# qingqing-zijin/LEAD-YOLO

Hardware: AMD Instinct MI355X
Metric: images/sec (640x640) fwd+bwd (higher is better)
Workload: dtype bf16; 1 GPU; lead-yolo-s bs=64/gpu 3x640x640 bf16 full train step: uint8 batch -> train-mode forward (batch-statistics BN), ComputeLoss, HIP backward, clip 10, SGD-nesterov 3 groups, ModelEMA update (BASELINE.json configs[2]); random-init weights; global_batch=64, parallelism=dp1 (single GPU, no collective), world_size=1

## Files before the change

### include/lead_yolo_hip.h

```cpp
#ifndef LEAD_YOLO_HIP_H
#define LEAD_YOLO_HIP_H
#ifdef __cplusplus
extern "C" {
#endif

enum { LY_F32 = 0, LY_BF16 = 1 };
int ly_abi_version(void);
const char* ly_last_error(void);

int ly_mlpblock_fwd(const void* x , void* y , int n_img, int H, int W, int C, const void* wp, const void* w1,
                    const void* w2, const float* bn_scale, const float* bn_shift, double* stats, int dtype, void* stream);
int ly_mlpblock_fwd_describe(int n_img, int H, int W, int C, int dtype, int with_stats , char* name, int cap);
int ly_mlpblock_pconv(const void* x , void* z , int n_img, int H, int W, int C, const void* wp, int dtype, void* stream);
int ly_mlpblock_pconv_describe(int n_img, int H, int W, int C, int dtype, char* name, int cap);
int ly_mlpblock_bwd_ok(int C, int dtype);
long ly_mlpblock_bwd_slab_floats(int C);
int ly_mlpblock_bwd(const void* x , const void* dy , void* g , int n_img, int H, int W, int C, const void* wp, const void* w1,
                    const void* w2t, const void* w1t, const float* a, const float* b, const float* alpha, const float* kappa, const float* lambda,
                    double* stats, float* slab, long slab_floats, float* dw1, float* dw2, int pass, int dtype, void* stream);
int ly_mlpblock_bwd_describe(int n_img, int H, int W, int C, int dtype, int pass, char* name, int cap);
int ly_mlpblock_bwd_dx_ok(int C, int W, int dtype);
int ly_mlpblock_bwd_dx(const void* g , const void* dy , const void* x , void* dx , int n_img, int H, int W, int C, const void* wpt,
                       float* slab, long slab_floats, float* dwp, int lddw, int dw_ts, int dw_cs, int dtype, void* stream);
int ly_mlpblock_bwd_dx_describe(int n_img, int H, int W, int C, int dtype, int with_dw , char* name, int cap);
// ... 52 lines not shown
} LyConv3Params;

int ly_conv3x3_fwd(const LyConv3Params* p, void* stream);
int ly_conv3x3_describe(const LyConv3Params* p, char* name, int cap);


int ly_pool_hw(const void* x , int ldx, int n_img, int H, int W, int C, float* pool, int dtype, void* stream);
int ly_coordatt_mlp(const float* pool, int n_img, int H, int W, int C, int mip, const float* w1, const float* b1,
                    const float* sc, const float* sh, const float* wh, const float* bh, const float* ww, const float* bw, float* a_h,
                    float* a_w, void* stream);
int ly_coordatt_mlp_bwd(const float* pool, int n_img, int H, int W, int C, int mip, const float* w1, const float* b1,
                        const float* mean, const float* invstd, const float* gamma, const float* beta, const float* wh,
                        const float* ww, const float* a_h, const float* a_w, const float* da_h, const float* da_w, float* ws,
                        double* sums , float* dpool, float* dw1, float* dgamma, float* dbeta, float* dwh, float* dbh, float* dww,
                        float* dbw, int grads_f64 , void* stream);

int ly_coordatt_gate(const void* x , int ldx, int n_img, int H, int W, int C, const float* a_h, const float* a_w,
                     const void* res , int ldres, void* out , int ldo, int dtype, void* stream);

int ly_se_fwd(const void* x , int ldx, int n_img, int HW, int C, const float* wa, const float* wb, int R, float* part,
              int slices, float* ca, int dtype, void* stream);
int ly_rfcbam_stats(const void* x , int ldx, int n_img, int H, int W, int C, int k, int s, const float* wg,
                    const float* a1, const float* b1, int TH, int TW, float* mm, float* part, int slices, int dtype, void* stream);
int ly_rfcbam_stats_describe(const void* x , int ldx, int n_img, int H, int W, int C, int k, int s, const float* wg, const float* a1, const float* b1,
                             int TH, int TW, float* mm, float* part, int slices, int dtype, char* name, int cap);
int ly_colsum(const void* x , int ldx, int n_img, int HW, int C, float* part, int slices, int dtype, void* stream);
int ly_rfcbam_mid(const float* part, int slices, int C, int HW, const float* wa, const float* wb, int R, float* ca, int n_img,
                  const float* mm, int HK, int WK, const float* w18, float* rfa, void* stream);
int ly_rfa_map(const float* mm, int n_img, int HK, int WK, const float* w, float* rfa, void* stream);

// ... 196 lines not shown
int ly_tune_wgrad3(int on);
int ly_tune_wgrad1(int on);

int ly_up2_bwd(const void* d , int ldd, int n_img, int Hs, int Ws, int C, void* out , int ldo, int dtype, void* stream);
int ly_unpatch(const void* g , int n_img, int Ho, int Wo, int C, int ks, void* dx , int dtype, void* stream);
int ly_sum_rows(const float* src, long R, long C, long ld, float* dst, int accumulate, void* stream);
int ly_patch4_rows_u8(const unsigned char* img, int n_img, int C, int H, int W, void* rows , int dtype, void* stream);
int ly_patch4_wgrad_u8(const unsigned char* img, int n_img, int C, int H, int W, const void* du , int lddu, int N, float scale, float* slab,
                       long slab_floats, float* dw , int dtype, void* stream);
int ly_patch4_wgrad_u8_describe(const unsigned char* img, int n_img, int C, int H, int W, const void* du , int lddu, int N, float scale, float* slab,
                                long slab_floats, float* dw, int dtype, char* name, int cap);

int ly_coordatt_gate_bwd(const void* dout , int ldd, const void* x , int ldx, int n_img, int H, int W, int C, const float* a_h,
                         const float* a_w, void* dx , int lddx, float* da_h, float* da_w, int bands, int slabs, int dtype, void* stream);
int ly_pool_hw_bwd(const float* gp, int n_img, int H, int W, int C, void* dx , int lddx, int accumulate, int dtype, void* stream);
int ly_maxpool_arg(const void* x , int ldx, int n_img, int H, int W, int C, int k, unsigned char* arg, int lda, int dtype, void* stream);
int ly_maxpool_gather(const unsigned char* arg, int lda, const float* d_up, int ldu, const void* d_own, int ldd, int own_dtype, int n_img, int H,
                      int W, int C, int k, void* out, int ldo, int out_dtype, void* stream);
int ly_sppf_bwd(const void* buf , int ldb, const void* d , int ldd, int n_img, int H, int W, int c, int k, void* out , int ldo, int dtype,
                void* stream);
int ly_mlp_dx(const void* dy , const void* g , const void* t , int ldt, long rows, int C, int c4, void* dx , int dtype, void* stream);
int ly_maxpool_bwd(const void* x , int ldx, const float* dy, int lddy, int n_img, int H, int W, int C, int k, float* dx, int lddx,
                   int dtype, void* stream);

int ly_rf_generate(const void* x , int ldx, int n_img, int H, int W, int C, int k, int s, const float* wg, void* ug , int dtype, void* stream);
int ly_rf_bwd_attn(int n_img, int H, int W, int C, int k, int s, const void* ug , const void* dcd , const float* ag, const float* bg,
                   const float* ca, const float* rfa, void* cd , float* d_rfa, float* gmax, float* d_ca, int dtype, void* stream);
int ly_rfa_bwd(const float* d_rfa, const float* rfa, const float* mm, const float* w18, int n_img, int Hk, int Wk, float* d_mm,
               float* dw18, int dw18_f64 , void* stream);
int ly_rf_bwd_relu(int n_img, int H, int W, int C, int k, int s, const void* ug , void* dcd , const float* ag, const float* bg,
// ... 110 lines not shown
```

### lead-yolo_amd/csrc/ly_attention.hip

```cpp
#include <float.h>

#include "ly_tile.hpp"
#include "ly_params.h"


template <typename T>
__global__ __launch_bounds__(LY_THREADS) void ly_pool_hw_kernel(const T* __restrict__ x, int ldx, int H, int W, int C,
                                                                 float* __restrict__ pool) {
  __shared__ f32x4 red[LY_THREADS];
  const int L = H + W;
  const int bid = ly_xcd_remap((int)blockIdx.x, (int)gridDim.x);
  const int n = bid / L, pos = bid - n * L;
  const int nc4 = C >> 2;
  const int tid = threadIdx.x;
  const int groups = LY_THREADS / nc4;
  const bool row = pos < H;
  const int len = row ? W : H;
  const long base = row ? ((long)n * H + pos) * W : ((long)n * H) * W + (pos - H);
  const long step = row ? 1 : W;
  const int c4 = tid % nc4, j0 = tid / nc4;
  f32x4 s = ly_zero4();
  if (j0 < groups) {
#pragma unroll 4
    for (int j = j0; j < len; j += groups) s += ly_ld4<T>(x + (base + j * step) * ldx + 4 * c4);
// ... 1231 lines not shown
                                                                                   n_img, H, W, C, Ho, Wo, s, mom)),
                                  "ly_rfcbam_tap_moments_kernel<%s>", ly_tname<T>()));
}

extern "C" int ly_rfcbam_tap_moments(const void* x, int ldx, int n_img, int H, int W, int C, int s, double* mom, int dtype, void* stream) {
  return tap_moments_entry(x, ldx, n_img, H, W, C, s, mom, dtype, LY_ON_STREAM(stream));
}

extern "C" int ly_rfcbam_tap_moments_describe(const void* x, int ldx, int n_img, int H, int W, int C, int s, double* mom, int dtype, char* name, int cap) {
  LY_CHECK(name && cap > 0, "rfcbam_tap_moments_describe: bad arguments");
  return tap_moments_entry(x, ldx, n_img, H, W, C, s, mom, dtype, LyOut{nullptr, name, cap});
}

__device__ __forceinline__ float ly_hswish_grad(float x) { return x <= -3.f ? 0.f : (x >= 3.f ? 1.f : (2.f * x + 3.f) * (1.f / 6.f)); }
#define LY_CA_STRIPES 32

template <int MIP, int NS>
__global__ __launch_bounds__(LY_THREADS) void ly_coordatt_mlp_bwd1_kernel(
    const float* __restrict__ pool, int n_img, int H, int W, int C, const float* __restrict__ w1, const float* __restrict__ b1,
    const float* __restrict__ mean, const float* __restrict__ invstd, const float* __restrict__ gamma, const float* __restrict__ beta,
    const float* __restrict__ wh, const float* __restrict__ ww, const float* __restrict__ a_h, const float* __restrict__ a_w,
    const float* __restrict__ da_h, const float* __restrict__ da_w, float* __restrict__ ws, double* __restrict__ sums, float* __restrict__ dzb) {
  const int tid = threadIdx.x, lane = tid & 63, wave = tid >> 6;
  const int L = H + W;
  const long R = (long)n_img * L;
  float s1 = 0.f, s2 = 0.f;
  static_assert(MIP == 8 || MIP == 16, "ly_coordatt_mlp_bwd1: MIP = 8 or 16");
  constexpr int LSTEP = 64 / MIP;
  const int mine = lane / LSTEP;
  const bool owner = (lane % LSTEP) == 0;
  const float b1m = b1[mine], meanm = mean[mine], invm = invstd[mine], gm = gamma[mine], bem = beta[mine];
  const long nw = (long)gridDim.x * 4;
  for (long r = (long)blockIdx.x * 4 + wave; r < R; r += nw) {
    const long n = r / L;
    const int pos = (int)(r - n * L);
    const bool isrow = pos < H;
    const long q = isrow ? n * H + pos : n * W + (pos - H);
    const float* wx = isrow ? wh : ww;
    const float* am = (isrow ? a_h : a_w) + q * C;
    const float* dam = (isrow ? da_h : da_w) + q * C;
    float y[MIP], d[MIP];
#pragma unroll
    for (int m = 0; m < MIP; ++m) { y[m] = 0.f; d[m] = 0.f; }
#pragma unroll
    for (int sl = 0; sl < NS; ++sl) {
      const int c = lane + 64 * sl;
      if (c < C) {
        const float pv = pool[r * C + c];
        const float av = am[c];
        const float dz = dam[c] * av * (1.f - av);
        dzb[r * C + c] = dz;
#pragma unroll
        for (int m = 0; m < MIP; ++m) {
          y[m] += w1[m * C + c] * pv;
          d[m] += dz * wx[c * MIP + m];
        }
      }
    }
    ly_reduce_scatter<MIP>(y, lane);
    ly_reduce_scatter<MIP>(d, lane);
    if (owner) {
      const float xh = (y[0] + b1m - meanm) * invm;
      const float y1 = gm * xh + bem;
      const float g = d[0] * ly_hswish_grad(y1);
      s1 += g;
// ... 91 lines not shown
    const int cl = e / NA, k = e - cl * NA;
    const int cc = blockIdx.x * 64 + cl;
    if (cc >= C) continue;
    const float v = red[e] + red[64 * NA + e] + red[2 * 64 * NA + e] + red[3 * 64 * NA + e];
    if (k < MIP) ly_gacc(dw1, k * C + cc, v, f64);
    else if (k < 2 * MIP) ly_gacc(dwh, cc * MIP + (k - MIP), v, f64);
    else if (k < 3 * MIP) ly_gacc(dww, cc * MIP + (k - 2 * MIP), v, f64);
    else if (k == 3 * MIP) ly_gacc(dbh, cc, v, f64);
    else ly_gacc(dbw, cc, v, f64);
  }
}

template <int MIP, int NS>
static void launch_coordatt_bwd(hipStream_t st, const float* pool, int n_img, int H, int W, int C, const float* w1, const float* b1, const float* mean,
                                const float* invstd, const float* gamma, const float* beta, const float* wh, const float* ww, const float* a_h,
                                const float* a_w, const float* da_h, const float* da_w, float* ws, double* sums, float* dpool, float* dw1,
                                float* dgamma, float* dbeta, float* dwh, float* dbh, float* dww, float* dbw, int f64) {
  const long R = (long)n_img * (H + W);
  long b1n = (R + 3) / 4;
  if (b1n > 1024) b1n = 1024;
  hipLaunchKernelGGL((ly_coordatt_mlp_bwd1_kernel<MIP, NS>), dim3((unsigned)b1n), dim3(LY_THREADS), 0, st, pool, n_img, H, W, C, w1, b1, mean, invstd, gamma,
                     beta, wh, ww, a_h, a_w, da_h, da_w, ws, sums, dpool);
  const int groups = (C + 63) / 64;
  long chunks = (96 + groups - 1) / groups;
  if (chunks > (R + 31) / 32) chunks = (R + 31) / 32;
  if (chunks < 1) chunks = 1;
  const long rpb = (R + chunks - 1) / chunks;
  chunks = (R + rpb - 1) / rpb;
  hipLaunchKernelGGL((ly_coordatt_mlp_bwd2_kernel<MIP>), dim3((unsigned)groups, (unsigned)chunks), dim3(LY_THREADS), 0, st, pool, n_img, H, W, C, rpb, w1,
                     gamma, invstd, ws, sums, dpool, dw1, dgamma, dbeta, dwh, dbh, dww, dbw, f64);
}

extern "C" int ly_coordatt_mlp_bwd(const float* pool, int n_img, int H, int W, int C, int mip, const float* w1, const float* b1,
                                   const float* mean, const float* invstd, const float* gamma, const float* beta, const float* wh,
                                   const float* ww, const float* a_h, const float* a_w, const float* da_h, const float* da_w, float* ws,
                                   double* sums, float* dpool, float* dw1, float* dgamma, float* dbeta, float* dwh, float* dbh,
                                   float* dww, float* dbw, int grads_f64, void* stream) {
  LY_CHECK(pool && w1 && b1 && mean && invstd && gamma && beta && wh && ww && a_h && a_w && da_h && da_w && ws && sums && dpool && dw1 &&
               dgamma && dbeta && dwh && dbh && dww && dbw, "coordatt_mlp_bwd: null pointer");
  LY_CHECK((mip == 8 || mip == 16) && C > 0 && C <= 512 && n_img > 0 && H > 0 && W > 0, "coordatt_mlp_bwd: built for mip 8 / 16 and C <= 512 (mip=%d C=%d)", mip, C);
  hipStream_t st = reinterpret_cast<hipStream_t>(stream);
#define LY_CA_BWD(MIP, NS) launch_coordatt_bwd<MIP, NS>(st, pool, n_img, H, W, C, w1, b1, mean, invstd, gamma, beta, wh, ww, a_h, a_w, da_h, da_w, ws, sums, \
                                                        dpool, dw1, dgamma, dbeta, dwh, dbh, dww, dbw, grads_f64)
  const int ns = (C + 63) / 64;
  if (mip == 8) {
    if (ns <= 1) LY_CA_BWD(8, 1); else if (ns <= 2) LY_CA_BWD(8, 2); else if (ns <= 4) LY_CA_BWD(8, 4); else LY_CA_BWD(8, 8);
  } else {
    if (ns <= 4) LY_CA_BWD(16, 4); else LY_CA_BWD(16, 8);
  }
#undef LY_CA_BWD
  LY_LAUNCH_CHECK();
  return 0;
}

__device__ __forceinline__ long ly_gw_index(int ch, int t, int e, int chunk, bool contiguous) {
  const int per = chunk >> 2;
  const int q = ch / chunk, r = ch - q * chunk;
  const int w = contiguous ? r / per : r & 3;
  const int j = contiguous ? r - w * per : r >> 2;
  const int p = j >> 1, ab = j & 1;
  return (((((long)q * 4 + w) * 9 + t) * (per >> 1) + p) * 10 + e) * 2 + ab;
}

__global__ __launch_bounds__(LY_THREADS) void ly_rfcbam_gen_prepare_kernel(
    const double* __restrict__ mom, int C, int KK, const float* __restrict__ gen_w, const float* __restrict__ gamma,
    const float* __restrict__ beta, float eps, float momentum, double count, float* __restrict__ running_mean,
    float* __restrict__ running_var, long* __restrict__ nbt, float* __restrict__ out8 , float* __restrict__ a1,
// ... 185 lines not shown
```

### lead-yolo_amd/csrc/ly_backward.hip

```cpp
#include "ly_tile.hpp"
#include "ly_params.h"

template <int ACT>
__device__ __forceinline__ f32x4 ly_dact4(const f32x4 v, const f32x4 dy) {
  f32x4 r;
#pragma unroll
  for (int i = 0; i < 4; ++i) {
    if (ACT == LY_ACT_RELU) {
      r[i] = v[i] > 0.f ? dy[i] : 0.f;
    } else if (ACT == LY_ACT_SILU) {
      const float s = ly_sigmoid(v[i]);
      r[i] = dy[i] * s * (1.f + v[i] * (1.f - s));
    } else {
      r[i] = dy[i];
    }
  }
  return r;
}

#ifndef LY_XCD_STREAM
#define LY_XCD_STREAM 1
#endif
#if LY_XCD_STREAM
#define LY_XCD_RANGE(total)                                                                                             \
// ... 451 lines not shown

extern "C" int ly_patch4_rows_u8(const unsigned char* img, int n_img, int C, int H, int W, void* rows, int dtype, void* stream) {
  LY_CHECK_DTYPE(dtype, "patch4_rows_u8");
  LY_CHECK(img && rows && n_img > 0 && C > 0 && C <= 16 && H > 0 && W > 0 && (H & 3) == 0 && (W & 3) == 0, "patch4_rows_u8: bad arguments");
  LY_CHECK(((uintptr_t)img & 3) == 0 && ((uintptr_t)rows & 15) == 0, "patch4_rows_u8: unaligned pointer");
  LY_CHECK((long)n_img * (H >> 2) < 65536, "patch4_rows_u8: too many patch rows");
  const dim3 grid((unsigned)(((W >> 2) + LY_P4_WO - 1) / LY_P4_WO), (unsigned)(n_img * (H >> 2)));
  LY_WITH_T(dtype, hipLaunchKernelGGL(ly_patch4_rows_u8_kernel<T>, grid, dim3(LY_THREADS), (size_t)LY_P4_WO * (16 * C + 8) * sizeof(T),
                                      reinterpret_cast<hipStream_t>(stream), img, C, H, W, reinterpret_cast<T*>(rows)));
  LY_LAUNCH_CHECK();
  return 0;
}

#define LY_CAG_RB 8
#define LY_CAG_MAXW 8
template <typename T>
__global__ __launch_bounds__(LY_THREADS) void ly_coordatt_gate_bwd_kernel(const T* __restrict__ dout, int ldd, const T* __restrict__ x,
                                                                           int ldx, int H, int W, int C, const float* __restrict__ a_h,
                                                                           const float* __restrict__ a_w, T* __restrict__ dx, int lddx,
                                                                           float* __restrict__ da_h, float* __restrict__ da_w, int bands, int slabs, long n_img) {
  __shared__ f32x4 red[LY_THREADS];
  const int nc4 = C >> 2, tid = threadIdx.x;
  const int groups = LY_THREADS / nc4;
  const int c4 = tid % nc4, g0 = tid / nc4;
  const int slab = blockIdx.x % slabs;
  const int bb = blockIdx.x / slabs;
  const long n = bb / bands;
  const int band = bb - (int)n * bands;
  const int w0 = slab * groups * LY_CAG_MAXW;
  const int h_lo = band * LY_CAG_RB, h_hi = h_lo + LY_CAG_RB < H ? h_lo + LY_CAG_RB : H;
  f32x4 accw[LY_CAG_MAXW], aw[LY_CAG_MAXW];
  bool okw[LY_CAG_MAXW];
  int wcl[LY_CAG_MAXW];
  const bool gok = g0 < groups;
#pragma unroll
// ... 11 lines not shown
    {
      const int c4c = gok ? c4 : 0;
      const f32x4 ah = ly_ldg4(a_h + nh * C + 4 * c4c);
      R4 dr[LY_CAG_MAXW], xr[LY_CAG_MAXW];
#pragma unroll
      for (int i = 0; i < LY_CAG_MAXW; ++i) {
        const long row = nh * W + wcl[i];
        dr[i] = ly_ldr4<T>(dout + row * ldd + 4 * c4c);
        xr[i] = ly_ldr4<T>(x + row * ldx + 4 * c4c);
      }
#pragma unroll
      for (int i = 0; i < LY_CAG_MAXW; ++i) {
        if (okw[i]) {
          const long row = nh * W + wcl[i];
          const f32x4 d = ly_r4_f32(dr[i]), xv = ly_r4_f32(xr[i]);
          ly_st4<T>(dx + row * lddx + 4 * c4, d * ah * aw[i]);
          const f32x4 t = d * xv;
          sh += t * aw[i];
          accw[i] += t * ah;
        }
      }
    }
    __syncthreads();
    red[tid] = sh;
    __syncthreads();
    if (g0 == 0) {
      for (int g = 1; g < groups; ++g) sh += red[g * nc4 + c4];
      ly_stg4(da_h + ((long)slab * n_img * H + nh) * C + 4 * c4, sh);
    }
  }
  if (g0 < groups) {
#pragma unroll
    for (int i = 0; i < LY_CAG_MAXW; ++i) {
      const int w = w0 + g0 + i * groups;
      if (w < W) {
        ly_stg4(da_w + ((long)band * n_img * W + n * W + w) * C + 4 * c4, accw[i]);
      }
    }
  }
}

extern "C" int ly_coordatt_gate_bwd(const void* dout, int ldd, const void* x, int ldx, int n_img, int H, int W, int C, const float* a_h,
                                    const float* a_w, void* dx, int lddx, float* da_h, float* da_w, int bands_in, int slabs_in, int dtype, void* stream) {
  LY_CHECK_DTYPE(dtype, "coordatt_gate_bwd");
  LY_CHECK(dout && x && a_h && a_w && dx && da_h && da_w, "coordatt_gate_bwd: null pointer");
  LY_CHECK((C & 3) == 0 && C <= 1024 && (ldd & 3) == 0 && (ldx & 3) == 0 && (lddx & 3) == 0, "coordatt_gate_bwd: C / ld must be multiples of 4");
  const int groups = LY_THREADS / (C >> 2);
  const int slabs = (W + groups * LY_CAG_MAXW - 1) / (groups * LY_CAG_MAXW);
  const int bands = (H + LY_CAG_RB - 1) / LY_CAG_RB;
  LY_CHECK(bands_in == bands && slabs_in == slabs, "coordatt_gate_bwd: the partial buffers are da_h [%d slabs][n][H][C] and da_w [%d bands][n][W][C] (got %d, %d)",
           slabs, bands, slabs_in, bands_in);
  LY_WITH_T(dtype, hipLaunchKernelGGL(ly_coordatt_gate_bwd_kernel<T>, dim3((unsigned)(n_img * bands * slabs)), dim3(LY_THREADS), 0, reinterpret_cast<hipStream_t>(stream),
                                      reinterpret_cast<const T*>(dout), ldd, reinterpret_cast<const T*>(x), ldx, H, W, C, a_h, a_w, reinterpret_cast<T*>(dx), lddx, da_h, da_w,
                                      bands, slabs, (long)n_img));
  LY_LAUNCH_CHECK();
  return 0;
}

template <typename T, bool ACC>
__global__ __launch_bounds__(LY_THREADS) void ly_pool_hw_bwd_kernel(const float* __restrict__ gp, int n_img, int H, int W, int C,
                                                                    T* __restrict__ dx, int lddx) {
  constexpr int VW = LyT<T>::VW, NQ = VW / 4;
  using RV = typename LyT<T>::RV;
  if ((C % VW) == 0 && (lddx % VW) == 0 && C / VW <= LY_THREADS) {
    const int ncv = C / VW, groups = LY_THREADS / ncv;
    const int cv = threadIdx.x % ncv, wl = threadIdx.x / ncv;
    if (wl >= groups) return;
    const int c = VW * cv;
    const float iw = 1.f / (float)W, ih = 1.f / (float)H;
// ... 40 lines not shown
}

extern "C" int ly_pool_hw_bwd(const float* gp, int n_img, int H, int W, int C, void* dx, int lddx, int accumulate, int dtype, void* stream) {
  LY_CHECK_DTYPE(dtype, "pool_hw_bwd");
  LY_CHECK(gp && dx && n_img > 0 && H > 0 && W > 0 && (C & 3) == 0 && (lddx & 3) == 0, "pool_hw_bwd: bad arguments");
  long nb = ly_ew_blocks((long)n_img * H * W * (C >> 2));
  if (nb > (long)n_img * H) nb = (long)n_img * H;
  const dim3 grid((unsigned)nb);
  if (accumulate) {
    LY_WITH_T(dtype, hipLaunchKernelGGL((ly_pool_hw_bwd_kernel<T, true>), grid, dim3(LY_THREADS), 0, reinterpret_cast<hipStream_t>(stream), gp, n_img, H, W, C,
                                        reinterpret_cast<T*>(dx), lddx));
  } else {
    LY_WITH_T(dtype, hipLaunchKernelGGL((ly_pool_hw_bwd_kernel<T, false>), grid, dim3(LY_THREADS), 0, reinterpret_cast<hipStream_t>(stream), gp, n_img, H, W, C,
                                        reinterpret_cast<T*>(dx), lddx));
  }
  LY_LAUNCH_CHECK();
  return 0;
}

template <typename T, int K>
__global__ __launch_bounds__(LY_THREADS) void ly_maxpool_bwd_kernel(const T* __restrict__ x, int ldx, const float* __restrict__ dy, int lddy,
                                                                    int n_img, int H, int W, int C, int k_rt, float* __restrict__ dx, int lddx) {
  const int nc4 = C >> 2;
  const int k = K > 0 ? K : k_rt, r = k >> 1;
  const long total = (long)n_img * H * W * nc4;
  for (long i = (long)blockIdx.x * LY_THREADS + threadIdx.x; i < total; i += (long)gridDim.x * LY_THREADS) {
    const long pix = i / nc4;
    const int c = 4 * (int)(i - pix * nc4);
    const long row = pix / W;
    const int w = (int)(pix - row * W);
// ... 575 lines not shown
```

### lead-yolo_amd/grad.py

```python
import collections
import ctypes
import functools

import os

import torch

from . import ops, pack
from .ops import ACT_NONE, ACT_RELU, ACT_SILU


_rows_dense = ops.rows_dense


FORK_SUM = True


class _Slot:
    __slots__ = ("deferred",)

    def __init__(self):
        self.deferred = []


# ... 551 lines not shown
    gp = ops.ParamGrad(p_wpc)
    dwp = gp.buf
    ts, cs = (c4, 1) if ops.tap_major(dwp) else (1, 9)
    wt = pack.packed(pack.src_taps(p_wpc, c4p, transposed_flipped=True), 9 * c4p, pl)
    dx, wdone = ops.mlpblock_bwd_dx(g, dy, x, n, h, w, c, wt, dwp=dwp, lddw=9 * c4, dw_ts=ts, dw_cs=cs)
    if not wdone:
        ops.wgrad(M=m, H=h, W=w, N=c4p, du=g, lddu=c, x=x, ldx=c, Hin=h, Win=w, Cin=c4p, dw=dwp, lddw=9 * c4, ks=3, stride=1, pad=1,
                  dw_ts=ts, dw_cs=cs, n_valid=c4, c_valid=c4)
    dwp, dw1, dw2 = gp.finish(), g1.finish(), g2.finish()
    return None, dx, dwp, dw1, dgamma, dbeta, dw2


MlpBlockFn._backward_fused = staticmethod(_mlpblock_backward_fused)


class CoordAttFn(torch.autograd.Function):

    @staticmethod
    def forward(ctx, mod, x, w1, b1, gamma, beta, wh, bh, ww, bw):
        t, ld = ops.rows(x)
        n, c, h, w = t.shape
        mip = mod.mip
        W1, Wh, Ww = (p.detach().reshape(p.shape[0], -1) for p in (w1, wh, ww))
        pool = ops.pool_hw(t, ld, n, h, w, c)
        st = ops.coordatt_conv1_stats(pool, n * (h + w), c, mip, W1, b1)
        sc, sh, mean, invstd = ops.bn_finalize(mod.bn1, st.view(1, -1), mip, n * (h + w), want_stats=True)
        a_h, a_w = ops.coordatt_mlp(pool, n, h, w, c, mip, W1, b1.detach(), Wh, bh.detach(), Ww, bw.detach(), sc=sc, sh=sh)
        out = ops.coordatt_gate(t, ld, n, h, w, c, a_h, a_w)
        ctx.save_for_backward(t, pool, a_h, a_w, mean, invstd)
        ctx.params = (w1, b1, gamma, beta, wh, bh, ww, bw)
        ctx.mip = mip
        return out

    @staticmethod
    def backward(ctx, dout):
        t, pool, a_h, a_w, mean, invstd = ctx.saved_tensors
        xr, ld = ops.rows(t)
        n, c, h, w = xr.shape
        w1, b1, gamma, beta, wh, bh, ww, bw = ctx.params
        dr, ldd = ops.rows(dout if dout.dtype == xr.dtype else dout.to(xr.dtype))
        dx, da_h, da_w = ops.coordatt_gate_bwd(dr, xr, ld, n, h, w, c, a_h, a_w, ldd=ldd)
        grads = ops.SmallGrad.group(ctx.params, zero=(1,))
        W1, Wh, Ww = (p.detach().reshape(p.shape[0], -1) for p in (w1, wh, ww))
        dpool = ops.coordatt_mlp_bwd(pool, n, h, w, c, ctx.mip, W1, b1.detach(), mean, invstd, gamma.detach(), beta.detach(), Wh, Ww, a_h, a_w,
                                     da_h, da_w, grads.bufs)
        ret = grads.values()
        ops.pool_hw_bwd(dpool, n, h, w, c, into=dx)
        grads.finish()
        return (None, dx, *ret)


def coordatt_train(mod, x):
    n, c, h, w = x.shape
    params = (mod.conv1.weight, mod.conv1.bias, mod.bn1.weight, mod.bn1.bias, mod.conv_h.weight, mod.conv_h.bias, mod.conv_w.weight, mod.conv_w.bias)
    width_ok = (mod.mip in (8, 16) and c <= 512) or not torch.is_grad_enabled()
    if width_ok and all(p is not None and p.dtype == torch.float32 for p in params):
        return CoordAttFn.apply(mod, x, *params)
    raise NotImplementedError(f"CoordAtt training is built for mip = max(8, c // 32) in (8, 16) and c <= 512 with float32 parameters (got mip={mod.mip}, "
                              f"c={c}): ly_coordatt_mlp_bwd has no instantiation for other widths, and there is no ATen fallback on the hot path")


class SppfPool(torch.autograd.Function):
# ... 331 lines not shown
```

### lead-yolo_amd/ops.py

```python
import ctypes
import os

import torch

from . import capi
from .capi import (ACT_NONE, ACT_RELU, ACT_SILU, GATHER_PATCH, GATHER_PATCH_NCHW, GATHER_PATCH_NCHW_BF16, GATHER_PATCH_NCHW_F16, GATHER_PATCH_NCHW_U8, GATHER_ROWS, GATHER_UP2,
                   PRO_AFFINE_RELU_CA, PRO_GATE, PRO_NONE)


PROFILE = None


class _Timed:

    def __init__(self, name, flops, nbytes, valu_flops=0.0):
        self.rec = None
        if PROFILE is not None:
            self.rec = [name, float(flops), float(nbytes), torch.cuda.Event(enable_timing=True), torch.cuda.Event(enable_timing=True), float(valu_flops)]

    def __enter__(self):
        if self.rec is not None:
            self.rec[3].record()

    def __exit__(self, *a):
# ... 233 lines not shown
def pool_hw(x, ldx, n, h, w, c):
    pool = torch.empty((n, h + w, c), dtype=torch.float32, device=x.device)
    with _Timed(f"ly_pool_hw_kernel<{_tname(x)}>", 1.0 * n * h * w * c, x.element_size() * n * h * w * c):
        capi.check(capi.lib().ly_pool_hw(_p(x), ldx, n, h, w, c, _p(pool), capi.dtype_code(x), capi.stream_ptr()), "ly_pool_hw")
    return pool


def coordatt_mlp(pool, n, h, w, c, mip, w1, b1, wh, bh, ww, bw, sc=None, sh=None):
    a_h = torch.empty((n, h, c), dtype=torch.float32, device=pool.device)
    a_w = torch.empty((n, w, c), dtype=torch.float32, device=pool.device)
    capi.check(capi.lib().ly_coordatt_mlp(_p(pool), n, h, w, c, mip, _p(w1), _p(b1), _p(sc), _p(sh), _p(wh), _p(bh), _p(ww), _p(bw), _p(a_h),
                                          _p(a_w), capi.stream_ptr()), "ly_coordatt_mlp")
    return a_h, a_w


def coordatt_mlp_bwd(pool, n, h, w, c, mip, w1, b1, mean, invstd, gamma, beta, wh, ww, a_h, a_w, da_h, da_w, targets):
    r = n * (h + w)
    sums = zeros_f64(32 * 2 * mip, pool.device)
    ws = torch.empty(r * 3 * mip, dtype=torch.float32, device=pool.device)
    dpool = torch.empty((n, h + w, c), dtype=torch.float32, device=pool.device)
    with _Timed(f"ly_coordatt_mlp_bwd2_kernel<{mip}>", 8.0 * r * c * mip, 4.0 * 4 * r * c):
        capi.check(capi.lib().ly_coordatt_mlp_bwd(_p(pool), n, h, w, c, mip, _p(w1), _p(b1), _p(mean), _p(invstd), _p(gamma), _p(beta), _p(wh), _p(ww),
                                                  _p(a_h), _p(a_w), _p(da_h), _p(da_w), _p(ws), _p(sums), _p(dpool),
                                                  *[_p(t) for t in targets], int(targets[0].dtype == torch.float64), capi.stream_ptr()),
                   "ly_coordatt_mlp_bwd")
    return dpool


def coordatt_gate(x, ldx, n, h, w, c, a_h, a_w, res=None, ldres=0):
    out = empty_nhwc(n, c, h, w, x)
    with _Timed(f"ly_gate_kernel<{_tname(x)}>", 2.0 * n * h * w * c, 2.0 * x.element_size() * n * h * w * c):
        capi.check(capi.lib().ly_coordatt_gate(_p(x), ldx, n, h, w, c, _p(a_h), _p(a_w), _p(res), ldres, _p(out), c, capi.dtype_code(x),
                                               capi.stream_ptr()), "ly_coordatt_gate")
    return out


def se_attention(x, ldx, n, hw, c, wa, wb, r, want_part=False):
    slices = se_slices(hw)
    part = torch.empty((n, slices, c), dtype=torch.float32, device=x.device)
    ca = torch.empty((n, c), dtype=torch.float32, device=x.device)
# ... 973 lines not shown
    ws = wgrad_workspace(img.device)
    return (img.dtype == torch.uint8 and img.is_contiguous() and c == 3 and h % 4 == 0 and w % 4 == 0 and du.dtype == torch.bfloat16
            and n_out % 8 == 0 and 8 <= n_out <= 64 and du.data_ptr() % 16 == 0 and ws is not None and ws.numel() >= 1536 * n_out * 48
            and n * (h // 4) * (w // 4) < (1 << 24))


def patch4_wgrad_u8(img, du, lddu, n_out, dw, scale):
    n, c, h, w = img.shape
    m = n * (h // 4) * (w // 4)
    ws = wgrad_workspace(img.device)
    args = (_p(img), n, c, h, w, _p(du), lddu, n_out, float(scale), _p(ws), ws.numel(), _p(dw), capi.dtype_code(du))
    with _Timed(_label("ly_patch4_wgrad_u8_describe", *args), 2.0 * m * n_out * 48, 1.0 * n * c * h * w + 2.0 * m * n_out + 4.0 * n_out * 48):
        capi.check(capi.lib().ly_patch4_wgrad_u8(*args, capi.stream_ptr()), "ly_patch4_wgrad_u8")


def coordatt_gate_bwd(dout, x, ldx, n, h, w, c, a_h, a_w, ldd=None):
    ldd = c if ldd is None else ldd
    dx = empty_nhwc(n, c, h, w, x)
    groups = 256 // (c // 4)
    slabs, bands = -(-w // (groups * 8)), -(-h // 8)
    ph = torch.empty((slabs, n * h * c), dtype=torch.float32, device=dout.device)
    pw = torch.empty((bands, n * w * c), dtype=torch.float32, device=dout.device)
    with _Timed(f"ly_coordatt_gate_bwd_kernel<{_tname(x)}>", 6.0 * n * h * w * c, 3.0 * x.element_size() * n * h * w * c):
        capi.check(capi.lib().ly_coordatt_gate_bwd(_p(dout), ldd, _p(x), ldx, n, h, w, c, _p(a_h), _p(a_w), _p(dx), c, _p(ph), _p(pw), bands, slabs,
                                                   capi.dtype_code(x), capi.stream_ptr()), "ly_coordatt_gate_bwd")
    da_h = (sum_rows(ph) if slabs > 1 else ph[0]).view(n, h, c)
    da_w = (sum_rows(pw) if bands > 1 else pw[0]).view(n, w, c)
    return dx, da_h, da_w


def pool_hw_bwd(gp, n, h, w, c, dtype=torch.float32, into=None):
    dx = into if into is not None else empty_nhwc(n, c, h, w, gp, dtype=dtype)
    capi.check(capi.lib().ly_pool_hw_bwd(_p(gp), n, h, w, c, _p(dx), c, 1 if into is not None else 0, capi.dtype_code(dx), capi.stream_ptr()),
               "ly_pool_hw_bwd")
    return dx


def maxpool_bwd(x, x_off, ldx, dy, dy_off, lddy, n, h, w, c, k, dx, dx_off, lddx):
    at = lambda t, off: ctypes.c_void_p(t.data_ptr() + t.element_size() * off)
    assert dy.dtype == torch.float32 and dx.dtype == torch.float32
    capi.check(capi.lib().ly_maxpool_bwd(at(x, x_off), ldx, at(dy, dy_off), lddy, n, h, w, c, k, at(dx, dx_off), lddx, capi.dtype_code(x),
                                         capi.stream_ptr()), "ly_maxpool_bwd")

# ... 49 lines not shown
```

Measured before the change: 7143 images/sec.

## Restructure CoordAtt backward: write dx once and fold partial sums inside MLP kernel

The CoordAtt backward used to write dx in the gate kernel and then read-modify-write it again in pool_hw_bwd, with separate sum_rows launches to reduce the da_h/da_w slab partials. Now the gate kernel only produces partial sums, and the MLP-backward kernel folds up to 12 partials inline. A new coordatt_dx kernel then writes dx = dout*a_h*a_w + pooled-gradient broadcast in a single pass. This removes the sum_rows launches and one full read-modify-write of dx, but dout is now read twice (once by the sums kernel and once by the dx kernel).

```diff
diff --git a/include/lead_yolo_hip.h b/include/lead_yolo_hip.h
--- a/include/lead_yolo_hip.h
+++ b/include/lead_yolo_hip.h
@@ -90,6 +90,11 @@
                         const float* ww, const float* a_h, const float* a_w, const float* da_h, const float* da_w, float* ws,
                         double* sums , float* dpool, float* dw1, float* dgamma, float* dbeta, float* dwh, float* dbh, float* dww,
                         float* dbw, int grads_f64 , void* stream);
+int ly_coordatt_mlp_bwd_parts(const float* pool, int n_img, int H, int W, int C, int mip, const float* w1, const float* b1,
+                              const float* mean, const float* invstd, const float* gamma, const float* beta, const float* wh,
+                              const float* ww, const float* a_h, const float* a_w, const float* da_h_part, int slabs, const float* da_w_part,
+                              int bands, float* ws, double* sums, float* dpool, float* dw1, float* dgamma, float* dbeta, float* dwh, float* dbh,
+                              float* dww, float* dbw, int grads_f64, void* stream);
 
 int ly_coordatt_gate(const void* x , int ldx, int n_img, int H, int W, int C, const float* a_h, const float* a_w,
                      const void* res , int ldres, void* out , int ldo, int dtype, void* stream);
@@ -316,6 +321,10 @@
 int ly_coordatt_gate_bwd(const void* dout , int ldd, const void* x , int ldx, int n_img, int H, int W, int C, const float* a_h,
                          const float* a_w, void* dx , int lddx, float* da_h, float* da_w, int bands, int slabs, int dtype, void* stream);
 int ly_pool_hw_bwd(const float* gp, int n_img, int H, int W, int C, void* dx , int lddx, int accumulate, int dtype, void* stream);
+int ly_coordatt_gate_bwd_sums(const void* dout , int ldd, const void* x , int ldx, int n_img, int H, int W, int C, const float* a_h,
+                              const float* a_w, float* da_h, float* da_w, int bands, int slabs, int dtype, void* stream);
+int ly_coordatt_dx(const void* dout , int ldd, int n_img, int H, int W, int C, const float* a_h, const float* a_w, const float* gp,
+                   void* dx , int lddx, int dtype, void* stream);
 int ly_maxpool_arg(const void* x , int ldx, int n_img, int H, int W, int C, int k, unsigned char* arg, int lda, int dtype, void* stream);
 int ly_maxpool_gather(const unsigned char* arg, int lda, const float* d_up, int ldu, const void* d_own, int ldd, int own_dtype, int n_img, int H,
                       int W, int C, int k, void* out, int ldo, int out_dtype, void* stream);
diff --git a/lead-yolo_amd/csrc/ly_attention.hip b/lead-yolo_amd/csrc/ly_attention.hip
--- a/lead-yolo_amd/csrc/ly_attention.hip
+++ b/lead-yolo_amd/csrc/ly_attention.hip
@@ -1269,16 +1269,55 @@
 
 __device__ __forceinline__ float ly_hswish_grad(float x) { return x <= -3.f ? 0.f : (x >= 3.f ? 1.f : (2.f * x + 3.f) * (1.f / 6.f)); }
 #define LY_CA_STRIPES 32
+#define LY_CA_MAX_PARTS 12
+
+template <int NP>
+__device__ __forceinline__ float ly_fold_parts_n(const float* __restrict__ p, const int R, const long ld) {
+  float v[NP];
+#pragma unroll
+  for (int k = 0; k < NP; ++k) v[k] = p[(k < R ? k : R - 1) * ld];
+  float a[4][4];
+  int m[4];
+#pragma unroll
+  for (int l = 0; l < 4; ++l) {
+    m[l] = ((R - l + 3) >> 2) & ~3;
+#pragma unroll
+    for (int e = 0; e < 4; ++e) a[l][e] = 0.f;
+  }
+#pragma unroll
+  for (int k = 0; k < NP; ++k) {
+    const int l = k & 3, j = k >> 2;
+    const float x = k < R ? v[k] : 0.f;
+    if ((j & 3) == 0) {
+      a[l][0] += x;
+    } else {
+      const bool tail = j >= m[l];
+      a[l][j & 3] += tail ? 0.f : x;
+      a[l][0] += tail ? x : 0.f;
+    }
+  }
+  float s = 0.f;
+#pragma unroll
+  for (int l = 0; l < 4; ++l) s += (a[l][0] + a[l][1]) + (a[l][2] + a[l][3]);
+  return s;
+}
+__device__ __forceinline__ float ly_fold_parts(const float* __restrict__ p, const int R, const long ld) {
+  if (R == 1) return p[0];
+  if (R <= 4) return ly_fold_parts_n<4>(p, R, ld);
+  return ly_fold_parts_n<LY_CA_MAX_PARTS>(p, R, ld);
+}
 
 template <int MIP, int NS>
 __global__ __launch_bounds__(LY_THREADS) void ly_coordatt_mlp_bwd1_kernel(
     const float* __restrict__ pool, int n_img, int H, int W, int C, const float* __restrict__ w1, const float* __restrict__ b1,
     const float* __restrict__ mean, const float* __restrict__ invstd, const float* __restrict__ gamma, const float* __restrict__ beta,
     const float* __restrict__ wh, const float* __restrict__ ww, const float* __restrict__ a_h, const float* __restrict__ a_w,
-    const float* __restrict__ da_h, const float* __restrict__ da_w, float* __restrict__ ws, double* __restrict__ sums, float* __restrict__ dzb) {
+    const float* __restrict__ da_h , const int nph, const float* __restrict__ da_w , const int npw,
+    float* __restrict__ ws, double* __restrict__ sums, float* __restrict__ dzb) {
   const int tid = threadIdx.x, lane = tid & 63, wave = tid >> 6;
   const int L = H + W;
   const long R = (long)n_img * L;
+  const long ldh = (long)n_img * H * C, ldw = (long)n_img * W * C;
   float s1 = 0.f, s2 = 0.f;
   static_assert(MIP == 8 || MIP == 16, "ly_coordatt_mlp_bwd1: MIP = 8 or 16");
   constexpr int LSTEP = 64 / MIP;
@@ -1294,6 +1333,8 @@
     const float* wx = isrow ? wh : ww;
     const float* am = (isrow ? a_h : a_w) + q * C;
     const float* dam = (isrow ? da_h : da_w) + q * C;
+    const int npart = isrow ? nph : npw;
+    const long ldpart = isrow ? ldh : ldw;
     float y[MIP], d[MIP];
 #pragma unroll
     for (int m = 0; m < MIP; ++m) { y[m] = 0.f; d[m] = 0.f; }
@@ -1303,7 +1344,7 @@
       if (c < C) {
         const float pv = pool[r * C + c];
         const float av = am[c];
-        const float dz = dam[c] * av * (1.f - av);
+        const float dz = ly_fold_parts(dam + c, npart, ldpart) * av * (1.f - av);
         dzb[r * C + c] = dz;
 #pragma unroll
         for (int m = 0; m < MIP; ++m) {
@@ -1425,13 +1466,13 @@
 template <int MIP, int NS>
 static void launch_coordatt_bwd(hipStream_t st, const float* pool, int n_img, int H, int W, int C, const float* w1, const float* b1, const float* mean,
                                 const float* invstd, const float* gamma, const float* beta, const float* wh, const float* ww, const float* a_h,
-                                const float* a_w, const float* da_h, const float* da_w, float* ws, double* sums, float* dpool, float* dw1,
+                                const float* a_w, const float* da_h, int nph, const float* da_w, int npw, float* ws, double* sums, float* dpool, float* dw1,
                                 float* dgamma, float* dbeta, float* dwh, float* dbh, float* dww, float* dbw, int f64) {
   const long R = (long)n_img * (H + W);
   long b1n = (R + 3) / 4;
   if (b1n > 1024) b1n = 1024;
   hipLaunchKernelGGL((ly_coordatt_mlp_bwd1_kernel<MIP, NS>), dim3((unsigned)b1n), dim3(LY_THREADS), 0, st, pool, n_img, H, W, C, w1, b1, mean, invstd, gamma,
-                     beta, wh, ww, a_h, a_w, da_h, da_w, ws, sums, dpool);
+                     beta, wh, ww, a_h, a_w, da_h, nph, da_w, npw, ws, sums, dpool);
   const int groups = (C + 63) / 64;
   long chunks = (96 + groups - 1) / groups;
   if (chunks > (R + 31) / 32) chunks = (R + 31) / 32;
@@ -1442,16 +1483,17 @@
                      gamma, invstd, ws, sums, dpool, dw1, dgamma, dbeta, dwh, dbh, dww, dbw, f64);
 }
 
-extern "C" int ly_coordatt_mlp_bwd(const float* pool, int n_img, int H, int W, int C, int mip, const float* w1, const float* b1,
-                                   const float* mean, const float* invstd, const float* gamma, const float* beta, const float* wh,
-                                   const float* ww, const float* a_h, const float* a_w, const float* da_h, const float* da_w, float* ws,
-                                   double* sums, float* dpool, float* dw1, float* dgamma, float* dbeta, float* dwh, float* dbh,
-                                   float* dww, float* dbw, int grads_f64, void* stream) {
+static int coordatt_mlp_bwd_entry(const float* pool, int n_img, int H, int W, int C, int mip, const float* w1, const float* b1, const float* mean,
+                                  const float* invstd, const float* gamma, const float* beta, const float* wh, const float* ww, const float* a_h,
+                                  const float* a_w, const float* da_h, int nph, const float* da_w, int npw, float* ws, double* sums, float* dpool,
+                                  float* dw1, float* dgamma, float* dbeta, float* dwh, float* dbh, float* dww, float* dbw, int grads_f64, void* stream) {
   LY_CHECK(pool && w1 && b1 && mean && invstd && gamma && beta && wh && ww && a_h && a_w && da_h && da_w && ws && sums && dpool && dw1 &&
                dgamma && dbeta && dwh && dbh && dww && dbw, "coordatt_mlp_bwd: null pointer");
   LY_CHECK((mip == 8 || mip == 16) && C > 0 && C <= 512 && n_img > 0 && H > 0 && W > 0, "coordatt_mlp_bwd: built for mip 8 / 16 and C <= 512 (mip=%d C=%d)", mip, C);
+  LY_CHECK(nph >= 1 && nph <= LY_CA_MAX_PARTS && npw >= 1 && npw <= LY_CA_MAX_PARTS, "coordatt_mlp_bwd: 1 .. %d partials of da_h / da_w are folded here (got %d, %d)",
+           LY_CA_MAX_PARTS, nph, npw);
   hipStream_t st = reinterpret_cast<hipStream_t>(stream);
-#define LY_CA_BWD(MIP, NS) launch_coordatt_bwd<MIP, NS>(st, pool, n_img, H, W, C, w1, b1, mean, invstd, gamma, beta, wh, ww, a_h, a_w, da_h, da_w, ws, sums, \
+#define LY_CA_BWD(MIP, NS) launch_coordatt_bwd<MIP, NS>(st, pool, n_img, H, W, C, w1, b1, mean, invstd, gamma, beta, wh, ww, a_h, a_w, da_h, nph, da_w, npw, ws, sums, \
                                                         dpool, dw1, dgamma, dbeta, dwh, dbh, dww, dbw, grads_f64)
   const int ns = (C + 63) / 64;
   if (mip == 8) {
@@ -1462,6 +1504,24 @@
 #undef LY_CA_BWD
   LY_LAUNCH_CHECK();
   return 0;
+}
+
+extern "C" int ly_coordatt_mlp_bwd(const float* pool, int n_img, int H, int W, int C, int mip, const float* w1, const float* b1,
+                                   const float* mean, const float* invstd, const float* gamma, const float* beta, const float* wh,
+                                   const float* ww, const float* a_h, const float* a_w, const float* da_h, const float* da_w, float* ws,
+                                   double* sums, float* dpool, float* dw1, float* dgamma, float* dbeta, float* dwh, float* dbh,
+                                   float* dww, float* dbw, int grads_f64, void* stream) {
+  return coordatt_mlp_bwd_entry(pool, n_img, H, W, C, mip, w1, b1, mean, invstd, gamma, beta, wh, ww, a_h, a_w, da_h, 1, da_w, 1, ws, sums, dpool, dw1, dgamma,
+                                dbeta, dwh, dbh, dww, dbw, grads_f64, stream);
+}
+
+extern "C" int ly_coordatt_mlp_bwd_parts(const float* pool, int n_img, int H, int W, int C, int mip, const float* w1, const float* b1,
+                                         const float* mean, const float* invstd, const float* gamma, const float* beta, const float* wh,
+                                         const float* ww, const float* a_h, const float* a_w, const float* da_h_part, int slabs,
+                                         const float* da_w_part, int bands, float* ws, double* sums, float* dpool, float* dw1, float* dgamma,
+                                         float* dbeta, float* dwh, float* dbh, float* dww, float* dbw, int grads_f64, void* stream) {
+  return coordatt_mlp_bwd_entry(pool, n_img, H, W, C, mip, w1, b1, mean, invstd, gamma, beta, wh, ww, a_h, a_w, da_h_part, slabs, da_w_part, bands, ws, sums, dpool,
+                                dw1, dgamma, dbeta, dwh, dbh, dww, dbw, grads_f64, stream);
 }
 
 __device__ __forceinline__ long ly_gw_index(int ch, int t, int e, int chunk, bool contiguous) {
diff --git a/lead-yolo_amd/csrc/ly_backward.hip b/lead-yolo_amd/csrc/ly_backward.hip
--- a/lead-yolo_amd/csrc/ly_backward.hip
+++ b/lead-yolo_amd/csrc/ly_backward.hip
@@ -489,11 +489,10 @@
 
 #define LY_CAG_RB 8
 #define LY_CAG_MAXW 8
-template <typename T>
-__global__ __launch_bounds__(LY_THREADS) void ly_coordatt_gate_bwd_kernel(const T* __restrict__ dout, int ldd, const T* __restrict__ x,
-                                                                           int ldx, int H, int W, int C, const float* __restrict__ a_h,
-                                                                           const float* __restrict__ a_w, T* __restrict__ dx, int lddx,
-                                                                           float* __restrict__ da_h, float* __restrict__ da_w, int bands, int slabs, long n_img) {
+template <typename T, bool DX>
+__device__ __forceinline__ void ly_coordatt_gate_bwd_body(const T* __restrict__ dout, int ldd, const T* __restrict__ x, int ldx, int H, int W, int C,
+                                                          const float* __restrict__ a_h, const float* __restrict__ a_w, T* __restrict__ dx, int lddx,
+                                                          float* __restrict__ da_h, float* __restrict__ da_w, int bands, int slabs, long n_img) {
   __shared__ f32x4 red[LY_THREADS];
   const int nc4 = C >> 2, tid = threadIdx.x;
   const int groups = LY_THREADS / nc4;
@@ -535,7 +534,7 @@
         if (okw[i]) {
           const long row = nh * W + wcl[i];
           const f32x4 d = ly_r4_f32(dr[i]), xv = ly_r4_f32(xr[i]);
-          ly_st4<T>(dx + row * lddx + 4 * c4, d * ah * aw[i]);
+          if constexpr (DX) ly_st4<T>(dx + row * lddx + 4 * c4, d * ah * aw[i]);
           const f32x4 t = d * xv;
           sh += t * aw[i];
           accw[i] += t * ah;
@@ -559,6 +558,20 @@
       }
     }
   }
+}
+template <typename T>
+__global__ __launch_bounds__(LY_THREADS) void ly_coordatt_gate_bwd_kernel(const T* __restrict__ dout, int ldd, const T* __restrict__ x,
+                                                                           int ldx, int H, int W, int C, const float* __restrict__ a_h,
+                                                                           const float* __restrict__ a_w, T* __restrict__ dx, int lddx,
+                                                                           float* __restrict__ da_h, float* __restrict__ da_w, int bands, int slabs, long n_img) {
+  ly_coordatt_gate_bwd_body<T, true>(dout, ldd, x, ldx, H, W, C, a_h, a_w, dx, lddx, da_h, da_w, bands, slabs, n_img);
+}
+template <typename T>
+__global__ __launch_bounds__(LY_THREADS) void ly_coordatt_gate_bwd_sums_kernel(const T* __restrict__ dout, int ldd, const T* __restrict__ x,
+                                                                                int ldx, int H, int W, int C, const float* __restrict__ a_h,
+                                                                                const float* __restrict__ a_w, float* __restrict__ da_h,
+                                                                                float* __restrict__ da_w, int bands, int slabs, long n_img) {
+  ly_coordatt_gate_bwd_body<T, false>(dout, ldd, x, ldx, H, W, C, a_h, a_w, nullptr, 0, da_h, da_w, bands, slabs, n_img);
 }
 
 extern "C" int ly_coordatt_gate_bwd(const void* dout, int ldd, const void* x, int ldx, int n_img, int H, int W, int C, const float* a_h,
@@ -574,6 +587,22 @@
   LY_WITH_T(dtype, hipLaunchKernelGGL(ly_coordatt_gate_bwd_kernel<T>, dim3((unsigned)(n_img * bands * slabs)), dim3(LY_THREADS), 0, reinterpret_cast<hipStream_t>(stream),
                                       reinterpret_cast<const T*>(dout), ldd, reinterpret_cast<const T*>(x), ldx, H, W, C, a_h, a_w, reinterpret_cast<T*>(dx), lddx, da_h, da_w,
                                       bands, slabs, (long)n_img));
+  LY_LAUNCH_CHECK();
+  return 0;
+}
+
+extern "C" int ly_coordatt_gate_bwd_sums(const void* dout, int ldd, const void* x, int ldx, int n_img, int H, int W, int C, const float* a_h,
+                                         const float* a_w, float* da_h, float* da_w, int bands_in, int slabs_in, int dtype, void* stream) {
+  LY_CHECK_DTYPE(dtype, "coordatt_gate_bwd_sums");
+  LY_CHECK(dout && x && a_h && a_w && da_h && da_w, "coordatt_gate_bwd_sums: null pointer");
+  LY_CHECK(C > 0 && (C & 3) == 0 && C <= 1024 && (ldd & 3) == 0 && (ldx & 3) == 0, "coordatt_gate_bwd_sums: C / ld must be multiples of 4");
+  const int groups = LY_THREADS / (C >> 2);
+  const int slabs = (W + groups * LY_CAG_MAXW - 1) / (groups * LY_CAG_MAXW);
+  const int bands = (H + LY_CAG_RB - 1) / LY_CAG_RB;
+  LY_CHECK(bands_in == bands && slabs_in == slabs, "coordatt_gate_bwd_sums: the partial buffers are da_h [%d slabs][n][H][C] and da_w [%d bands][n][W][C] (got %d, %d)",
+           slabs, bands, slabs_in, bands_in);
+  LY_WITH_T(dtype, hipLaunchKernelGGL(ly_coordatt_gate_bwd_sums_kernel<T>, dim3((unsigned)(n_img * bands * slabs)), dim3(LY_THREADS), 0, reinterpret_cast<hipStream_t>(stream),
+                                      reinterpret_cast<const T*>(dout), ldd, reinterpret_cast<const T*>(x), ldx, H, W, C, a_h, a_w, da_h, da_w, bands, slabs, (long)n_img));
   LY_LAUNCH_CHECK();
   return 0;
 }
@@ -644,6 +673,96 @@
     LY_WITH_T(dtype, hipLaunchKernelGGL((ly_pool_hw_bwd_kernel<T, false>), grid, dim3(LY_THREADS), 0, reinterpret_cast<hipStream_t>(stream), gp, n_img, H, W, C,
                                         reinterpret_cast<T*>(dx), lddx));
   }
+  LY_LAUNCH_CHECK();
+  return 0;
+}
+
+__device__ __forceinline__ f32x4 ly_fma4(const f32x4 a, const f32x4 b, const f32x4 c) {
+  return (f32x4){__builtin_fmaf(a.x, b.x, c.x), __builtin_fmaf(a.y, b.y, c.y), __builtin_fmaf(a.z, b.z, c.z), __builtin_fmaf(a.w, b.w, c.w)};
+}
+__device__ __forceinline__ f32x4 ly_opaque4(f32x4 v) {
+  asm("" : "+v"(v));
+  return v;
+}
+template <typename T>
+__global__ __launch_bounds__(LY_THREADS) void ly_coordatt_dx_kernel(const T* __restrict__ dout, int ldd, int n_img, int H, int W, int C,
+                                                                    const float* __restrict__ a_h, const float* __restrict__ a_w,
+                                                                    const float* __restrict__ gp, T* __restrict__ dx, int lddx, const int vec) {
+  constexpr int VW = LyT<T>::VW, NQ = VW / 4;
+  using RV = typename LyT<T>::RV;
+  const float iw = 1.f / (float)W, ih = 1.f / (float)H;
+  if (vec) {
+    const int ncv = C / VW, groups = LY_THREADS / ncv;
+    const int cv = threadIdx.x % ncv, wl = threadIdx.x / ncv;
+    if (wl >= groups) return;
+    const int c = VW * cv;
+    const long rows = (long)n_img * H;
+    for (long nh = blockIdx.x; nh < rows; nh += gridDim.x) {
+      const long n = nh / H;
+      const int h = (int)(nh - n * H);
+      const float* const ga = gp + (n * (H + W) + h) * C + c;
+      const float* const gb = gp + (n * (H + W) + H) * C + c;
+      const float* const awp = a_w + n * W * C + c;
+      f32x4 a[NQ], ah[NQ];
+#pragma unroll
+      for (int q = 0; q < NQ; ++q) {
+        a[q] = ly_ldg4(ga + 4 * q) * iw;
+        ah[q] = ly_ldg4(a_h + nh * C + c + 4 * q);
+      }
+      const T* const srow = dout + nh * (long)W * ldd + c;
+      T* const drow = dx + nh * (long)W * lddx + c;
+      for (int w = wl; w < W; w += groups) {
+        f32x4 d[NQ], o[NQ], v[NQ];
+        ly_rv_unpack(ly_ldrv<T>(srow + (long)w * ldd), d);
+#pragma unroll
+        for (int q = 0; q < NQ; ++q) {
+          d[q] = d[q] * ah[q] * ly_ldg4(awp + (long)w * C + 4 * q);
+          v[q] = ly_fma4(ly_ldg4(gb + (long)w * C + 4 * q), (f32x4){ih, ih, ih, ih}, a[q]);
+        }
+        ly_rv_unpack(ly_rv_pack(d, (RV*)nullptr), o);
+#pragma unroll
+        for (int q = 0; q < NQ; ++q) v[q] += ly_opaque4(o[q]);
+        *reinterpret_cast<RV*>(drow + (long)w * lddx) = ly_rv_pack(v, (RV*)nullptr);
+      }
+    }
+  } else {
+    using R4 = typename LyT<T>::R4;
+    const int nc4 = C >> 2;
+    const long total = (long)n_img * H * W * nc4;
+    for (long i = (long)blockIdx.x * LY_THREADS + threadIdx.x; i < total; i += (long)gridDim.x * LY_THREADS) {
+      const long pix = i / nc4;
+      const int c = 4 * (int)(i - pix * nc4);
+      const long row = pix / W;
+      const int w = (int)(pix - row * W);
+      const long n = row / H;
+      const int h = (int)(row - n * H);
+      const f32x4 a = ly_ldg4(gp + (n * (H + W) + h) * C + c), b = ly_ldg4(gp + (n * (H + W) + H + w) * C + c);
+      const f32x4 d = ly_r4_f32(ly_ldr4<T>(dout + pix * ldd + c));
+      const f32x4 g = d * ly_ldg4(a_h + row * C + c) * ly_ldg4(a_w + (n * W + w) * C + c);
+      R4 r;
+      ly_st4<T>(reinterpret_cast<T*>(&r), g);
+      f32x4 v = ly_fma4(a, (f32x4){iw, iw, iw, iw}, b * ih);
+      v += ly_opaque4(ly_r4_f32(r));
+      ly_st4<T>(dx + pix * lddx + c, v);
+    }
+  }
+}
+
+extern "C" int ly_coordatt_dx(const void* dout, int ldd, int n_img, int H, int W, int C, const float* a_h, const float* a_w, const float* gp,
+                              void* dx, int lddx, int dtype, void* stream) {
+  LY_CHECK_DTYPE(dtype, "coordatt_dx");
+  LY_CHECK(dout && a_h && a_w && gp && dx, "coordatt_dx: null pointer");
+  LY_CHECK(n_img > 0 && H > 0 && W > 0 && C > 0 && (C & 3) == 0 && ldd >= C && lddx >= C && (ldd & 3) == 0 && (lddx & 3) == 0, "coordatt_dx: bad arguments");
+  const int vw = dtype == LY_BF16 ? 8 : 4;
+  const uintptr_t a4 = dtype == LY_BF16 ? 8 : 16;
+  LY_CHECK(((uintptr_t)dout % a4) == 0 && ((uintptr_t)dx % a4) == 0, "coordatt_dx: dout / dx must be aligned to 4 elements");
+  const bool vec = (C % vw) == 0 && (ldd % vw) == 0 && (lddx % vw) == 0 && C / vw <= LY_THREADS && ((uintptr_t)dout & 15) == 0 && ((uintptr_t)dx & 15) == 0;
+  long nb = ly_ew_blocks((long)n_img * H * W * (C >> 2));
+  if (vec && nb > (long)n_img * H) nb = (long)n_img * H;
+  const dim3 grid((unsigned)nb);
+  hipStream_t st = reinterpret_cast<hipStream_t>(stream);
+  LY_WITH_T(dtype, hipLaunchKernelGGL(ly_coordatt_dx_kernel<T>, grid, dim3(LY_THREADS), 0, st, reinterpret_cast<const T*>(dout), ldd, n_img, H, W, C, a_h, a_w, gp,
+                                      reinterpret_cast<T*>(dx), lddx, (int)vec));
   LY_LAUNCH_CHECK();
   return 0;
 }
diff --git a/lead-yolo_amd/grad.py b/lead-yolo_amd/grad.py
--- a/lead-yolo_amd/grad.py
+++ b/lead-yolo_amd/grad.py
@@ -589,6 +589,10 @@
 MlpBlockFn._backward_fused = staticmethod(_mlpblock_backward_fused)
 
 
+CA_BWD_DX_ONCE = True
+CA_BWD_FOLD_IN_MLP = True
+
+
 class CoordAttFn(torch.autograd.Function):
 
     @staticmethod
@@ -614,13 +618,18 @@
         n, c, h, w = xr.shape
         w1, b1, gamma, beta, wh, bh, ww, bw = ctx.params
         dr, ldd = ops.rows(dout if dout.dtype == xr.dtype else dout.to(xr.dtype))
-        dx, da_h, da_w = ops.coordatt_gate_bwd(dr, xr, ld, n, h, w, c, a_h, a_w, ldd=ldd)
+        dx, ph, pw = ops.coordatt_gate_bwd_parts(dr, xr, ld, n, h, w, c, a_h, a_w, ldd=ldd, want_dx=not CA_BWD_DX_ONCE)
+        parts = CA_BWD_FOLD_IN_MLP and max(ph.shape[0], pw.shape[0]) <= ops.CA_MAX_PARTS
+        da_h, da_w = (ph, pw) if parts else ops.coordatt_fold_parts(ph, pw, n, h, w, c)
         grads = ops.SmallGrad.group(ctx.params, zero=(1,))
         W1, Wh, Ww = (p.detach().reshape(p.shape[0], -1) for p in (w1, wh, ww))
         dpool = ops.coordatt_mlp_bwd(pool, n, h, w, c, ctx.mip, W1, b1.detach(), mean, invstd, gamma.detach(), beta.detach(), Wh, Ww, a_h, a_w,
-                                     da_h, da_w, grads.bufs)
+                                     da_h, da_w, grads.bufs, parts=parts)
         ret = grads.values()
-        ops.pool_hw_bwd(dpool, n, h, w, c, into=dx)
+        if dx is None:
+            dx = ops.coordatt_dx(dr, ldd, n, h, w, c, a_h, a_w, dpool)
+        else:
+            ops.pool_hw_bwd(dpool, n, h, w, c, into=dx)
         grads.finish()
         return (None, dx, *ret)
 
diff --git a/lead-yolo_amd/ops.py b/lead-yolo_amd/ops.py
--- a/lead-yolo_amd/ops.py
+++ b/lead-yolo_amd/ops.py
@@ -271,16 +271,18 @@
     return a_h, a_w
 
 
-def coordatt_mlp_bwd(pool, n, h, w, c, mip, w1, b1, mean, invstd, gamma, beta, wh, ww, a_h, a_w, da_h, da_w, targets):
+def coordatt_mlp_bwd(pool, n, h, w, c, mip, w1, b1, mean, invstd, gamma, beta, wh, ww, a_h, a_w, da_h, da_w, targets, parts=False):
     r = n * (h + w)
     sums = zeros_f64(32 * 2 * mip, pool.device)
     ws = torch.empty(r * 3 * mip, dtype=torch.float32, device=pool.device)
     dpool = torch.empty((n, h + w, c), dtype=torch.float32, device=pool.device)
+    head = (_p(pool), n, h, w, c, mip, _p(w1), _p(b1), _p(mean), _p(invstd), _p(gamma), _p(beta), _p(wh), _p(ww), _p(a_h), _p(a_w))
+    tail = (_p(ws), _p(sums), _p(dpool), *[_p(t) for t in targets], int(targets[0].dtype == torch.float64), capi.stream_ptr())
     with _Timed(f"ly_coordatt_mlp_bwd2_kernel<{mip}>", 8.0 * r * c * mip, 4.0 * 4 * r * c):
-        capi.check(capi.lib().ly_coordatt_mlp_bwd(_p(pool), n, h, w, c, mip, _p(w1), _p(b1), _p(mean), _p(invstd), _p(gamma), _p(beta), _p(wh), _p(ww),
-                                                  _p(a_h), _p(a_w), _p(da_h), _p(da_w), _p(ws), _p(sums), _p(dpool),
-                                                  *[_p(t) for t in targets], int(targets[0].dtype == torch.float64), capi.stream_ptr()),
-                   "ly_coordatt_mlp_bwd")
+        if parts:
+            capi.check(capi.lib().ly_coordatt_mlp_bwd_parts(*head, _p(da_h), da_h.shape[0], _p(da_w), da_w.shape[0], *tail), "ly_coordatt_mlp_bwd_parts")
+        else:
+            capi.check(capi.lib().ly_coordatt_mlp_bwd(*head, _p(da_h), _p(da_w), *tail), "ly_coordatt_mlp_bwd")
     return dpool
 
 
@@ -1284,19 +1286,44 @@
         capi.check(capi.lib().ly_patch4_wgrad_u8(*args, capi.stream_ptr()), "ly_patch4_wgrad_u8")
 
 
-def coordatt_gate_bwd(dout, x, ldx, n, h, w, c, a_h, a_w, ldd=None):
+CA_MAX_PARTS = 12
+
+
+def coordatt_gate_bwd_parts(dout, x, ldx, n, h, w, c, a_h, a_w, ldd=None, want_dx=True):
     ldd = c if ldd is None else ldd
-    dx = empty_nhwc(n, c, h, w, x)
     groups = 256 // (c // 4)
     slabs, bands = -(-w // (groups * 8)), -(-h // 8)
     ph = torch.empty((slabs, n * h * c), dtype=torch.float32, device=dout.device)
     pw = torch.empty((bands, n * w * c), dtype=torch.float32, device=dout.device)
-    with _Timed(f"ly_coordatt_gate_bwd_kernel<{_tname(x)}>", 6.0 * n * h * w * c, 3.0 * x.element_size() * n * h * w * c):
-        capi.check(capi.lib().ly_coordatt_gate_bwd(_p(dout), ldd, _p(x), ldx, n, h, w, c, _p(a_h), _p(a_w), _p(dx), c, _p(ph), _p(pw), bands, slabs,
-                                                   capi.dtype_code(x), capi.stream_ptr()), "ly_coordatt_gate_bwd")
-    da_h = (sum_rows(ph) if slabs > 1 else ph[0]).view(n, h, c)
-    da_w = (sum_rows(pw) if bands > 1 else pw[0]).view(n, w, c)
-    return dx, da_h, da_w
+    if want_dx:
+        dx = empty_nhwc(n, c, h, w, x)
+        with _Timed(f"ly_coordatt_gate_bwd_kernel<{_tname(x)}>", 6.0 * n * h * w * c, 3.0 * x.element_size() * n * h * w * c):
+            capi.check(capi.lib().ly_coordatt_gate_bwd(_p(dout), ldd, _p(x), ldx, n, h, w, c, _p(a_h), _p(a_w), _p(dx), c, _p(ph), _p(pw), bands, slabs,
+                                                       capi.dtype_code(x), capi.stream_ptr()), "ly_coordatt_gate_bwd")
+        return dx, ph, pw
+    with _Timed(f"ly_coordatt_gate_bwd_sums_kernel<{_tname(x)}>", 4.0 * n * h * w * c, 2.0 * x.element_size() * n * h * w * c):
+        capi.check(capi.lib().ly_coordatt_gate_bwd_sums(_p(dout), ldd, _p(x), ldx, n, h, w, c, _p(a_h), _p(a_w), _p(ph), _p(pw), bands, slabs,
+                                                        capi.dtype_code(x), capi.stream_ptr()), "ly_coordatt_gate_bwd_sums")
+    return None, ph, pw
+
+
+def coordatt_fold_parts(ph, pw, n, h, w, c):
+    da_h = (sum_rows(ph) if ph.shape[0] > 1 else ph[0]).view(n, h, c)
+    da_w = (sum_rows(pw) if pw.shape[0] > 1 else pw[0]).view(n, w, c)
+    return da_h, da_w
+
+
+def coordatt_gate_bwd(dout, x, ldx, n, h, w, c, a_h, a_w, ldd=None):
+    dx, ph, pw = coordatt_gate_bwd_parts(dout, x, ldx, n, h, w, c, a_h, a_w, ldd=ldd)
+    return (dx, *coordatt_fold_parts(ph, pw, n, h, w, c))
+
+
+def coordatt_dx(dout, ldd, n, h, w, c, a_h, a_w, gp):
+    dx = empty_nhwc(n, c, h, w, dout)
+    with _Timed(f"ly_coordatt_dx_kernel<{_tname(dout)}>", 4.0 * n * h * w * c, 2.0 * dout.element_size() * n * h * w * c):
+        capi.check(capi.lib().ly_coordatt_dx(_p(dout), ldd, n, h, w, c, _p(a_h), _p(a_w), _p(gp), _p(dx), c, capi.dtype_code(dout), capi.stream_ptr()),
+                   "ly_coordatt_dx")
+    return dx
 
 
 def pool_hw_bwd(gp, n, h, w, c, dtype=torch.float32, into=None):
```

Result: no change. 7169 images/sec (median of 6 runs) (+0.4%).
